# cyberfabric/cyberfabric-core

Hardware: NVIDIA H100
Metric: prompt_bytes_per_sec_bpe_encode (higher is better)
Workload: dtype u32

## Files before the change

### cyberfabric-core_b200/csrc/bpe_kernels.cuh

```cuda
#pragma once
#include <stdint.h>

#include "pretok.cuh"
#include "pretok_fsm.h"
#include "pretok_sync.cuh"
#include "specials.h"
#include "tables.h"
#include "tma.cuh"

namespace cfbpe {

#ifdef CUSIM_EMULATOR
#define CFBPE_DYN_SMEM(name) uint32_t* const name = reinterpret_cast<uint32_t*>(cusim::dyn_smem())
#else
#define CFBPE_DYN_SMEM(name) extern __shared__ __align__(16) uint32_t name[]
#endif

constexpr uint32_t kMaxVocabs = 8;
#ifdef CUSIM_EMULATOR
inline unsigned long long* dbg_counters() { static unsigned long long c[16]; return c; }
#define CFBPE_DBG_COUNT(i) (++dbg_counters()[i])
#else
#define CFBPE_DBG_COUNT(i) ((void)0)
#endif

#ifndef CFBPE_SPLIT_CHUNK
#define CFBPE_SPLIT_CHUNK 64
#endif
constexpr uint32_t kSplitChunk = CFBPE_SPLIT_CHUNK;
constexpr uint32_t kBigPiece = 256;
constexpr uint32_t kScanTileWords = 256;

struct VocabSet {
    TablesView v[kMaxVocabs];
    uint32_t loaded_mask;
};

struct BatchView {
    const uint8_t* bytes;
    const uint64_t* offsets;
    const uint8_t* vocab_ids;
    uint32_t n_prompts;
    uint64_t total_bytes;
};

struct DeviceStatus {
    uint32_t bad_utf8;
    uint32_t n_long;
    uint32_t long_overflow;
    uint32_t long_next;
    uint32_t n_big;
    uint32_t defer_next;
    uint64_t n_tokens;
    uint64_t tok_end;
    unsigned long long long_bytes;
    unsigned long long long_tokens;
    uint32_t miss_n[3];
    uint32_t miss_next[3];
    uint32_t miss_overflow;
    uint32_t extra_n;
    uint32_t split_next;
    uint32_t fix_n;
    uint32_t bad_vocab;
    uint32_t defer_n;
    unsigned long long defer_parts;
    uint64_t n_chunks;
    uint64_t chunk_end;
};

struct MissLists {
    uint64_t* list[3];
    uint32_t cap[3];
};
__host__ __device__ inline uint32_t miss_class_min_len(uint32_t c) { return c == 0 ? 13u : (c == 1 ? 7u : 1u); }

struct LongPiece { uint64_t start; uint64_t end; uint32_t vocab; uint32_t pad; };

__device__ __forceinline__ uint32_t find_prompt(const uint64_t* __restrict__ offsets, uint32_t n, uint64_t pos) {
    uint32_t lo = 0, hi = n;
    while (hi - lo > 1) {
        const uint32_t mid = (lo + hi) >> 1;
        if (offsets[mid] <= pos) lo = mid; else hi = mid;
    }
    return lo;
}

__device__ __forceinline__ void or_bits(uint32_t* __restrict__ words, uint64_t word, uint32_t bits) {
    if (bits) atomicOr(&words[word], bits);
}

__device__ __forceinline__ void prefetch_l2(const void* p) {
#if !defined(CUSIM_EMULATOR)
    asm volatile("prefetch.global.L2 [%0];" ::"l"(p));
#else
    (void)p;
#endif
}

__device__ __forceinline__ uint64_t same_byte_run_end(const uint8_t* __restrict__ s, uint64_t pos, uint64_t pe, uint32_t c) {
    uint64_t e = pos;
    while (e < pe && (reinterpret_cast<uintptr_t>(s + e) & 15u)) { if (s[e] != c) return e; ++e; }
    const uint32_t w = c * 0x01010101u;
    for (uint64_t a = e; a < pe && a < e + 1024; a += 128) prefetch_l2(s + a);
    while (e + 128 <= pe) {
        if (e + 1024 < pe) prefetch_l2(s + e + 1024);
        uint4 v[8];
// ... 513 lines not shown
    uint32_t* sid = &s_id[wic][0][lane];
    uint32_t* srk = &s_rk[wic][0][lane];
    if (status->miss_overflow) return;
    TablesView T = vs.v[0];
    uint32_t vid = 0;
#pragma unroll 1
    for (uint32_t c = 0; c < 3; ++c) {
        const uint32_t n = status->miss_n[c];
        const uint64_t* __restrict__ list = ml.list[c];
        for (;;) {
            uint32_t t0 = 0;
            if (lane == 0) t0 = atomicAdd(&status->miss_next[c], 32u);
            t0 = __shfl_sync(kFull, t0, 0);
            if (t0 >= n) break;
            const uint32_t i = t0 + lane;
            uint32_t alive = 0, rank = 0;
            if (i < n) {
                const uint64_t e = list[i];
                const uint64_t pos = e & 0xFFFFFFFFull;
                rank = static_cast<uint32_t>(e >> 32);
                const uint64_t end = next_set_bit(piece_bits, pos + 1, b.total_bytes);
                if (multi) {
                    const uint32_t pv = b.vocab_ids[find_prompt(b.offsets, b.n_prompts, pos)];
                    if (pv != vid) { vid = pv; T = vs.v[vid]; }
                }
                alive = merge_piece_in_lane(T, text, pos, static_cast<uint32_t>(end - pos), sid, srk, tok_bits);
            }
            const uint32_t cnt = __popc(alive);
            uint32_t incl = cnt;
#pragma unroll
            for (uint32_t d = 1; d < 32; d <<= 1) { const uint32_t o = __shfl_up_sync(kFull, incl, d); if (lane >= d) incl += o; }
            const uint32_t total = __shfl_sync(kFull, incl, 31);
            uint32_t base = 0;
            if (lane == 0 && total) base = atomicAdd(&status->extra_n, total);
            base = __shfl_sync(kFull, base, 0);
            if (cnt) {
                uint32_t slot = base + incl - cnt;
                if (slot + cnt <= dn.extras_cap) {
                    dn.by_piece[rank] = kPieceMulti | slot;
                    for (uint32_t bits = alive; bits; bits &= bits - 1) dn.extras[slot++] = sid[(static_cast<uint32_t>(__ffs(bits)) - 1u) * 32];
                } else atomicOr(&status->miss_overflow, 1u);
            }
            __syncwarp();
        }
    }
}

struct LongScratch {
    uint32_t* rank;
    uint32_t* aux0;
    uint32_t* aux1;
};

__device__ __forceinline__ uint32_t warp_min_u32(uint32_t v) {
#pragma unroll
    for (uint32_t d = 16; d; d >>= 1) { const uint32_t o = __shfl_xor_sync(kFull, v, d); v = o < v ? o : v; }
    return v;
}

__device__ __forceinline__ bool select_chunk(uint32_t r, uint32_t rmin, uint32_t lane, uint32_t& carry, uint32_t& sel_ballot) {
    const bool cand = (r == rmin);
    const uint32_t C = __ballot_sync(kFull, cand);
    const uint32_t z = ~C & lanemask_lt(lane);
    const uint32_t s = z ? (32u - __clz(z)) : 0u;
    const uint32_t cnt = lane - s + (s == 0 ? carry : 0u);
    const bool sel = cand && !(cnt & 1u);
    sel_ballot = __ballot_sync(kFull, sel);
    const uint32_t nz = ~C;
    carry = nz ? static_cast<uint32_t>(__clz(nz)) : (carry + 32u);
    return sel;
}

__device__ __forceinline__ void array_round(const TablesView& T, uint32_t* id, uint32_t* rk, uint32_t* a0, uint32_t* a1,
                                            uint32_t m, uint32_t rmin, uint32_t lane) {
    uint32_t carry = 0, prevS = 0, cut = kNone;
    for (uint32_t base = 0; base < m && cut == kNone; base += 32) {
        const uint32_t i = base + lane;
        const uint32_t r = (i + 1 < m) ? rk[i] : kNone;
        uint32_t S;
        const bool sel = select_chunk(r, rmin, lane, carry, S);
        bool viol = false;
        if (sel) {
            const bool selm2 = (lane >= 2) ? ((S >> (lane - 2)) & 1u) : ((prevS >> (30 + lane)) & 1u);
            uint32_t L = kNone, R = kNone;
            if (i > 0) L = pair_lookup(T, selm2 ? rmin : id[i - 1], rmin);
            if (i + 2 < m) R = pair_lookup(T, rmin, id[i + 2]);
            a0[i] = L;
            a1[i] = R;
            viol = (L < rmin) || (R < rmin);
        }
        const uint32_t V = __ballot_sync(kFull, viol);
        if (V) cut = base + (__ffs(V) - 1);
        prevS = S;
    }
    __syncwarp();
    carry = 0; prevS = 0;
    for (uint32_t base = 0; base < m && base <= cut; base += 32) {
        const uint32_t i = base + lane;
        const uint32_t r = (i + 1 < m) ? rk[i] : kNone;
        uint32_t S;
        const bool sel = select_chunk(r, rmin, lane, carry, S);
        const bool app = sel && i <= cut;
        const bool selm2 = (lane >= 2) ? ((S >> (lane - 2)) & 1u) : ((prevS >> (30 + lane)) & 1u);
        uint32_t L = kNone;
        if (app) {
            L = a0[i];
            id[i] = rmin;
            id[i + 1] = kNone;
            rk[i] = a1[i];
        }
        __syncwarp();
        if (app && i > 0) rk[selm2 ? i - 2 : i - 1] = L;
        __syncwarp();
        prevS = S;
    }
}
template <uint32_t kPosBits>
__device__ __forceinline__ uint32_t array_compact(uint32_t* id, uint32_t* rk, uint32_t m, uint32_t lane, uint32_t& rmin_out) {
    uint32_t out = 0, nmin = kNone;
    for (uint32_t base = 0; base < m; base += 32) {
        const uint32_t i = base + lane;
        const uint32_t myid = (i < m) ? id[i] : kNone;
        uint32_t myrk = (i < m) ? rk[i] : kNone;
        if (kPosBits && myrk != kNone) myrk >>= kPosBits;
        const bool keep = myid != kNone;
        const uint32_t K = __ballot_sync(kFull, keep);
        const uint32_t pos = out + __popc(K & lanemask_lt(lane));
        __syncwarp();
        if (keep) { id[pos] = myid; rk[pos] = myrk; nmin = myrk < nmin ? myrk : nmin; }
        out += __popc(K);
    }
    __syncwarp();
    rmin_out = warp_min_u32(nmin);
    return out;
}

constexpr uint32_t kListMax = 65535;
constexpr uint32_t kMedSmem = 256;

__device__ __forceinline__ bool key_less(uint32_t r1, uint32_t p1, uint32_t r2, uint32_t p2) { return r1 < r2 || (r1 == r2 && p1 < p2); }

__device__ __forceinline__ void list_rounds_multi(const TablesView& T, uint32_t* id, uint32_t* rk, uint32_t* link, uint32_t* nid,
                                                  uint32_t m, uint32_t lane) {
    constexpr uint32_t kNoPrev = 0xFFFFu;
    for (uint32_t i = lane; i < m; i += 32) {
        link[i] = ((i + 1) << 16) | (i ? i - 1 : kNoPrev);
        nid[i] = (i + 1 < m) ? id[i + 1] : kNone;
    }
    __syncwarp();
    const uint32_t c = ((m + 31) / 32) | 1u;
    const uint32_t lo = lane * c < m ? lane * c : m;
    const uint32_t hi = lo + c < m ? lo + c : m;
    for (;;) {
        uint32_t m1 = kNone, p1 = 0, m2 = kNone, p2 = 0;
        for (uint32_t xb = lo; xb < hi; xb += 16) {
            uint32_t v[16];
#pragma unroll
            for (uint32_t t = 0; t < 16; ++t) v[t] = (xb + t < hi) ? rk[xb + t] : kNone;
#pragma unroll
            for (uint32_t t = 0; t < 16; ++t) {
                if (v[t] < m1) { m2 = m1; p2 = p1; m1 = v[t]; p1 = xb + t; }
                else if (v[t] < m2) { m2 = v[t]; p2 = xb + t; }
            }
        }
        if (!__any_sync(kFull, m1 != kNone)) break;
        const bool valid = m1 != kNone;
        const uint32_t x = p1, r = m1;
        uint32_t j = 0, q = kNoPrev, k = m, L = kNone, R = kNone;
        if (valid) {
            const uint32_t li = link[x];
            j = li >> 16; q = li & 0xFFFFu;
            k = link[j] >> 16;
            const uint32_t idk = nid[j];
            const uint32_t idq = (q != kNoPrev) ? id[q] : 0u;
// ... 107 lines not shown
                if (R != kNone) Rk = (R << kPosBits) | x;
                if (L != kNone) Lk = (L << kPosBits) | q;
            }
            have = dirty != nullptr;
        }
        const bool valid = m1 != kNoKey;
        const uint32_t x = m1 & kPosMask, r = m1 >> kPosBits;
        uint32_t v = kNoKey;
        bool viol = false;
        if (valid) {
            uint32_t cc = m2 < Lk ? m2 : Lk;
            cc = cc < Rk ? cc : Rk;
            viol = cc <= m1;
            v = cc > m1 + 1u ? cc : m1 + 1u;
            if (v == kNoKey) v = kNoKey - 1u;
            atomicMin(&claim[x], m1);
            atomicMin(&claim[j], m1);
        }
        group_sync();
        if (kWarps > 1 && tid == 0) eq_flag[(round + 1u) & 1u] = 0;
        if (valid) {
            uint32_t lowest = claim[x];
            const uint32_t cj = claim[j];
            lowest = cj < lowest ? cj : lowest;
            if (q != kNoPrev) { const uint32_t cq = claim[q]; lowest = cq < lowest ? cq : lowest; }
            if (k < m) { const uint32_t ck = claim[k]; lowest = ck < lowest ? ck : lowest; }
            if (lowest < m1) { v = m1; have = false; }
        }
        uint32_t cut = __reduce_min_sync(kFull, v);
        if (kWarps > 1) {
            uint32_t* red = s_red + (round & 1u) * kWarps;
            if (lane == 0) red[wid] = cut;
            __syncthreads();
            cut = red[0];
#pragma unroll
            for (uint32_t w = 1; w < kWarps; ++w) { const uint32_t o = red[w]; cut = o < cut ? o : cut; }
        } else {
            __syncwarp();
        }
        if (cut == kNoKey) return true;
        if (kWarps > 1 && tid == 0) CFBPE_DBG_COUNT(6);
        if (kWarps > 1 && valid && m1 < cut) CFBPE_DBG_COUNT(7);
        bool eq = valid && m1 < cut && !viol && (cut >> kPosBits) == (m1 >> kPosBits);
        if (kWarps == 1) eq = __any_sync(kFull, eq);
        else if (eq) eq_flag[round & 1u] = 1u;
        if (valid) {
            claim[x] = kNoKey; claim[j] = kNoKey;
            if (m1 < cut) {
                id[x] = r; id[j] = kNone;
                kk[j] = kNoKey; kk[x] = Rk;
                link[x] = (k << 16) | q;
                if (k < m) link[k] = (link[k] & 0xFFFF0000u) | x;
                if (q != kNoPrev) kk[q] = Lk;
                have = false;
                if (dirty) {
                    if (j >= hi) dirty[(j * inv_c) >> 20] = 1u;
                    if (q != kNoPrev && q < lo) dirty[(q * inv_c) >> 20] = 1u;
                }
            }
        }
        group_sync();
        if (kWarps > 1) eq = eq_flag[round & 1u] != 0u;
        eq_run = eq ? eq_run + 1u : 0u;
        if (eq_run >= 3u) {
            const uint32_t er = cut >> kPosBits;
            uint32_t cnt = 0;
            for (uint32_t y = lo; y < hi; ++y) cnt += (kk[y] >> kPosBits) == er ? 1u : 0u;
            cnt = __reduce_add_sync(kFull, cnt);
            if (kWarps > 1) {
                uint32_t* sum = s_red + 2 * kWarps + 2;
                if (lane == 0) sum[wid] = cnt;
                __syncthreads();
                cnt = 0;
#pragma unroll
                for (uint32_t w = 0; w < kWarps; ++w) cnt += sum[w];
                __syncthreads();
            }
            if (cnt >= 8u && cnt * 32u >= m) return false;
            eq_run = 0;
        }
    }
}

__device__ __forceinline__ void flag_parts(const uint32_t* id, uint32_t* copy_to, uint32_t m, uint64_t start,
                                           uint32_t* __restrict__ tok_bits, DeviceStatus* status, uint32_t lane) {
    for (uint32_t base = 0; base < m; base += 32) {
        const uint32_t i = base + lane;
        const uint32_t v = (i < m) ? id[i] : kNone;
        const bool alive = v != kNone;
        if (alive && copy_to) copy_to[i] = v;
        const uint32_t A = __ballot_sync(kFull, alive);
        if (lane == 0 && A) {
            atomicAdd(&status->long_tokens, static_cast<unsigned long long>(__popc(A)));
            const uint64_t pos = start + base;
            const uint32_t sh = static_cast<uint32_t>(pos & 31);
            atomicOr(&tok_bits[pos >> 5], A << sh);
            if (sh && (A >> (32 - sh))) atomicOr(&tok_bits[(pos >> 5) + 1], A >> (32 - sh));
        }
    }
}

constexpr uint32_t kDeferMaxParts = 4096;
constexpr uint32_t kListSmemBytes = kDeferMaxParts * 16;
constexpr uint32_t kListMaxRank = (1u << 20) - 1u;
__device__ __forceinline__ bool list_kernel_takes(const TablesView& T, uint32_t n_bytes) { return n_bytes <= kDeferMaxParts && T.n_ranks < kListMaxRank; }


constexpr uint32_t kLongWarps = 4;
#ifndef CFBPE_LONG_MIN_CTAS
#define CFBPE_LONG_MIN_CTAS (32 / kLongWarps)
#endif
__global__ void __launch_bounds__(kLongWarps * 32, CFBPE_LONG_MIN_CTAS)
bpe_long_kernel(BatchView b, VocabSet vs, LongPiece* long_list, DeviceStatus* status,
                uint32_t long_cap, uint32_t* __restrict__ ids_by_pos, LongScratch sc, uint32_t* __restrict__ tok_bits) {
    __shared__ uint32_t s_med[kLongWarps][4][kMedSmem];
    const uint32_t lane = threadIdx.x & 31;
    const uint32_t n_big = status->n_big;
    const uint32_t n_all = status->long_overflow ? 0u : status->n_long + n_big;
    for (;;) {
        uint32_t item = 0;
        if (lane == 0) item = atomicAdd(&status->long_next, 1u);
        item = __shfl_sync(kFull, item, 0);
        if (item >= n_all) break;
        const uint32_t slot = item < n_big ? long_cap - 1 - item : item - n_big;
        const LongPiece lp = long_list[slot];
        const TablesView T = vs.v[lp.vocab];
        const uint8_t* __restrict__ p = b.bytes + lp.start;
        const uint32_t n = static_cast<uint32_t>(lp.end - lp.start);
#ifndef CFBPE_NO_DEFER
        if (item < n_big && list_kernel_takes(T, n)) continue;
#endif
        uint32_t* const gid = ids_by_pos + lp.start;
        const bool in_smem = n <= kMedSmem;
        uint32_t* id = in_smem ? s_med[threadIdx.x >> 5][0] : gid;
        uint32_t* rk = in_smem ? s_med[threadIdx.x >> 5][1] : sc.rank + lp.start;
        uint32_t* a0 = in_smem ? s_med[threadIdx.x >> 5][2] : sc.aux0 + lp.start;
        uint32_t* a1 = in_smem ? s_med[threadIdx.x >> 5][3] : sc.aux1 + lp.start;

        if (n <= T.max_token_len) {
            uint32_t t = kNone;
            if (lane == 0) t = piece_lookup(T, p, n);
            t = __shfl_sync(kFull, t, 0);
            if (t != kNone) {
                if (lane == 0) { gid[0] = t; atomicOr(&tok_bits[lp.start >> 5], 1u << (lp.start & 31)); atomicAdd(&status->long_tokens, 1ull); }
                continue;
            }
        }
        uint32_t m = n;
        uint32_t rmin = kNone;
        for (uint32_t i = lane; i < n; i += 32) {
            const uint32_t c0 = p[i];
            id[i] = T.byte2id[c0];
            const uint32_t r = (i + 1 < n) ? T.bytepair[(c0 << 8) | p[i + 1]] : kNone;
            rk[i] = r;
            rmin = r < rmin ? r : rmin;
        }
        rmin = warp_min_u32(rmin);
        __syncwarp();

        bool deferred = false;
        while (rmin != kNone) {
            array_round(T, id, rk, a0, a1, m, rmin, lane);
            const uint32_t before = m;
            m = array_compact<0>(id, rk, m, lane, rmin);
            const uint32_t merged = before - m;
            if (rmin == kNone || merged * 8u >= m || m <= 32u || m > kListMax) continue;
            if (in_smem) {
                if (list_rounds_par<1, 8>(T, id, rk, a0, a1, m, nullptr)) break;
                if (lane == 0) CFBPE_DBG_COUNT(1);
                m = array_compact<8>(id, rk, m, lane, rmin);
                continue;
            }
            if (lane == 0) CFBPE_DBG_COUNT(5);
            list_rounds_multi(T, id, rk, a0, a1, m, lane);
            __syncwarp();
            break;
        }
        if (deferred) continue;
        __syncwarp();
        flag_parts(id, in_smem ? gid : nullptr, m, lp.start, tok_bits, status, lane);
        __syncwarp();
    }
}

constexpr uint32_t kCtaChunk = 16;

__device__ __forceinline__ void cta_array_round(const TablesView& T, uint32_t* id, uint32_t* rk, uint32_t* a0, uint32_t* a1,
                                                uint32_t m, uint32_t rmin, uint32_t* s_scan, uint32_t* s_sel) {
    const uint32_t P = blockDim.x, t = threadIdx.x;
    const uint32_t c = (m + P - 1) / P;
    const uint32_t lo = t * c < m ? t * c : m, hi = lo + c < m ? lo + c : m;
    uint32_t tail = 0, all = 1;
    for (uint32_t i = lo; i < hi; ++i) {
        const bool cand = (i + 1 < m) && rk[i] == rmin;
        if (cand) ++tail; else { tail = 0; all = 0; }
    }
    s_scan[t] = (all << 31) | tail;
    if (t == 0) s_scan[P] = kNone;
    for (uint32_t w = t; w < kDeferMaxParts / 32; w += P) s_sel[w] = 0;
    __syncthreads();
    uint32_t cnt = 0;
    for (uint32_t u = t; u > 0 && lo < m;) {
        const uint32_t e = s_scan[--u];
        cnt += e & 0x7FFFFFFFu;
        if (!(e >> 31)) break;
    }
    uint32_t sel_bits = 0;
    for (uint32_t i = lo; i < hi; ++i) {
        const bool cand = (i + 1 < m) && rk[i] == rmin;
        if (cand && !(cnt & 1u)) { sel_bits |= 1u << (i - lo); atomicOr(&s_sel[i >> 5], 1u << (i & 31)); }
        cnt = cand ? cnt + 1 : 0;
    }
    __syncthreads();
    uint32_t m2_bits = 0;
    for (uint32_t bts = sel_bits; bts; bts &= bts - 1) {
        const uint32_t k = static_cast<uint32_t>(__ffs(bts)) - 1u, i = lo + k;
        const bool selm2 = i >= 2 && ((s_sel[(i - 2) >> 5] >> ((i - 2) & 31)) & 1u);
        uint32_t L = kNone, R = kNone;
        if (i > 0) L = pair_lookup(T, selm2 ? rmin : id[i - 1], rmin);
        if (i + 2 < m) R = pair_lookup(T, rmin, id[i + 2]);
        a0[i] = L; a1[i] = R;
        if (selm2) m2_bits |= 1u << k;
        if (L < rmin || R < rmin) atomicMin(&s_scan[P], i);
    }
    __syncthreads();
    const uint32_t cut = s_scan[P];
    for (uint32_t bts = sel_bits; bts; bts &= bts - 1) {
        const uint32_t i = lo + static_cast<uint32_t>(__ffs(bts)) - 1u;
        if (i > cut) break;
        id[i] = rmin; id[i + 1] = kNone; rk[i] = a1[i];
    }
    __syncthreads();
    for (uint32_t bts = sel_bits; bts; bts &= bts - 1) {
        const uint32_t k = static_cast<uint32_t>(__ffs(bts)) - 1u, i = lo + k;
        if (i > cut) break;
        if (i > 0) rk[((m2_bits >> k) & 1u) ? i - 2 : i - 1] = a0[i];
    }
    __syncthreads();
}

template <uint32_t kPosBits>
__device__ __forceinline__ uint32_t cta_array_compact(uint32_t* id, uint32_t* rk, uint32_t m, uint32_t& rmin_out, uint32_t* s_scan) {
    const uint32_t P = blockDim.x, t = threadIdx.x, lane = t & 31u, wid = t >> 5;
    const uint32_t c = (m + P - 1) / P;
    const uint32_t lo = t * c < m ? t * c : m, hi = lo + c < m ? lo + c : m;
    uint32_t vid[kCtaChunk], vrk[kCtaChunk];
    uint32_t keep = 0, nmin = kNone;
#pragma unroll
    for (uint32_t k = 0; k < kCtaChunk; ++k) {
        const uint32_t i = lo + k;
        vid[k] = (k < c && i < hi) ? id[i] : kNone;
        uint32_t r = (k < c && i < hi) ? rk[i] : kNone;
        if (kPosBits && r != kNone) r >>= kPosBits;
        vrk[k] = r;
        if (vid[k] != kNone) { ++keep; nmin = r < nmin ? r : nmin; }
    }
    uint32_t x = keep;
#pragma unroll
    for (uint32_t d = 1; d < 32; d <<= 1) { const uint32_t o = __shfl_up_sync(kFull, x, d); if (lane >= d) x += o; }
    nmin = warp_min_u32(nmin);
    if (lane == 31) s_scan[wid] = x;
    if (lane == 0) s_scan[32 + wid] = nmin;
    __syncthreads();
    uint32_t woff = 0, total = 0, rmin = kNone;
    for (uint32_t w = 0; w < (P >> 5); ++w) { const uint32_t v = s_scan[w]; if (w < wid) woff += v; total += v; const uint32_t r = s_scan[32 + w]; rmin = r < rmin ? r : rmin; }
    uint32_t pos = woff + x - keep;
#pragma unroll
    for (uint32_t k = 0; k < kCtaChunk; ++k) if (vid[k] != kNone) { id[pos] = vid[k]; rk[pos] = vrk[k]; ++pos; }
    __syncthreads();
    rmin_out = rmin;
    return total;
}

#ifndef CFBPE_LIST_WARPS
#define CFBPE_LIST_WARPS 8
#endif
constexpr uint32_t kListWarps = CFBPE_LIST_WARPS;
static_assert(kListWarps * 32 * kCtaChunk >= kDeferMaxParts, "a thread's chunk of the batched rounds holds kCtaChunk parts");

__global__ void __launch_bounds__(kListWarps * 32, 3)
bpe_list_kernel(BatchView b, VocabSet vs, const LongPiece* __restrict__ long_list, DeviceStatus* status,
                uint32_t long_cap, uint32_t* __restrict__ ids_by_pos, LongScratch sc, uint32_t* __restrict__ tok_bits) {
    CFBPE_DYN_SMEM(s_dyn);
    __shared__ uint32_t s_red[3 * kListWarps + 2];
    __shared__ uint32_t s_item, s_tok;
    __shared__ uint32_t s_dirty[kListWarps * 32];
    __shared__ uint32_t s_scan[kListWarps * 32 + 64];
    __shared__ uint32_t s_sel[kDeferMaxParts / 32];
    const uint32_t n_big = status->long_overflow ? 0u : status->n_big;
    uint32_t* const id = s_dyn;
    uint32_t* const kk = s_dyn + kDeferMaxParts;
    uint32_t* const link = s_dyn + 2 * kDeferMaxParts;
    uint32_t* const claim = s_dyn + 3 * kDeferMaxParts;
    (void)sc;
    for (;;) {
        if (threadIdx.x == 0) s_item = atomicAdd(&status->defer_next, 1u);
        __syncthreads();
        const uint32_t item = s_item;
        __syncthreads();
        if (item >= n_big) break;
        const LongPiece lp = long_list[long_cap - 1 - item];
        const TablesView T = vs.v[lp.vocab];
        const uint32_t n = static_cast<uint32_t>(lp.end - lp.start);
        if (!list_kernel_takes(T, n)) continue;
        const uint8_t* __restrict__ p = b.bytes + lp.start;
        uint32_t* const gid = ids_by_pos + lp.start;
        if (n <= T.max_token_len) {
            if (threadIdx.x == 0) s_tok = piece_lookup(T, p, n);
            __syncthreads();
            const uint32_t tok = s_tok;
            __syncthreads();
            if (tok != kNone) {
                if (threadIdx.x == 0) { gid[0] = tok; atomicOr(&tok_bits[lp.start >> 5], 1u << (lp.start & 31)); atomicAdd(&status->long_tokens, 1ull); }
                continue;
            }
        }
        uint32_t m = n, rmin = kNone;
        for (uint32_t i = threadIdx.x; i < n; i += kListWarps * 32) {
            const uint32_t c0 = p[i];
            id[i] = T.byte2id[c0];
            const uint32_t r = (i + 1 < n) ? T.bytepair[(c0 << 8) | p[i + 1]] : kNone;
            kk[i] = r;
            rmin = r < rmin ? r : rmin;
        }
        rmin = warp_min_u32(rmin);
        if ((threadIdx.x & 31) == 0) s_scan[threadIdx.x >> 5] = rmin;
        __syncthreads();
        rmin = kNone;
        for (uint32_t w = 0; w < kListWarps; ++w) { const uint32_t r = s_scan[w]; rmin = r < rmin ? r : rmin; }
        __syncthreads();
        bool counted = false;
        while (rmin != kNone) {
            cta_array_round(T, id, kk, link, claim, m, rmin, s_scan, s_sel);
            const uint32_t before = m;
            m = cta_array_compact<0>(id, kk, m, rmin, s_scan);
            if (rmin == kNone || (before - m) * 8u >= m || m <= 32u) continue;
            if (!counted && threadIdx.x == 0) { atomicAdd(&status->defer_n, 1u); atomicAdd(&status->defer_parts, static_cast<unsigned long long>(m)); CFBPE_DBG_COUNT(0); }
            counted = true;
            const bool done = list_rounds_par<kListWarps, 12>(T, id, kk, link, claim, m, s_red, s_dirty);
            __syncthreads();
            if (done) break;
            if (threadIdx.x == 0) CFBPE_DBG_COUNT(2);
            m = cta_array_compact<12>(id, kk, m, rmin, s_scan);
        }
        __syncthreads();
        if (threadIdx.x < 32) flag_parts(id, gid, m, lp.start, tok_bits, status, threadIdx.x);
        __syncthreads();
    }
}

__device__ __forceinline__ uint32_t block_reduce_add_256(uint32_t v, uint32_t* s_tmp) {
#pragma unroll
    for (uint32_t d = 16; d; d >>= 1) v += __shfl_xor_sync(kFull, v, d);
    if ((threadIdx.x & 31) == 0) s_tmp[threadIdx.x >> 5] = v;
    __syncthreads();
    uint32_t t = 0;
    for (uint32_t w = 0; w < (blockDim.x + 31) / 32; ++w) t += s_tmp[w];
    __syncthreads();
    return t;
}

__global__ void __launch_bounds__(256)
flag_count_kernel(uint32_t* __restrict__ tok_bits, const uint32_t* __restrict__ piece_bits, uint64_t n_words, uint32_t* __restrict__ tile_counts) {
    __shared__ uint32_t s_tmp[8];
    const uint64_t base = static_cast<uint64_t>(blockIdx.x) * kScanTileWords;
    uint32_t c = 0;
    for (uint32_t i = threadIdx.x; i < kScanTileWords; i += blockDim.x) {
        const uint64_t w = base + i;
        if (w < n_words) { const uint32_t t = tok_bits[w], f = t | piece_bits[w]; if (f != t) tok_bits[w] = f; c += __popc(f); }
    }
    const uint32_t t = block_reduce_add_256(c, s_tmp);
    if (threadIdx.x == 0) tile_counts[blockIdx.x] = t;
}

__global__ void __launch_bounds__(1024)
tile_scan_kernel(const uint32_t* __restrict__ tile_counts, uint32_t n_tiles, uint64_t* __restrict__ tile_base,
                 DeviceStatus* status, const uint64_t* __restrict__ token_base) {
    __shared__ uint64_t s_warp[32];
    const uint64_t base0 = token_base ? *token_base : 0;
    const uint32_t lane = threadIdx.x & 31, wid = threadIdx.x >> 5, nwarps = (blockDim.x + 31) >> 5;
    const uint32_t per = ((n_tiles + nwarps - 1) / nwarps + 31u) & ~31u;
    const uint32_t lo = wid * per < n_tiles ? wid * per : n_tiles;
    const uint32_t hi = lo + per < n_tiles ? lo + per : n_tiles;
    uint64_t sum = 0;
    for (uint32_t i = lo + lane; i < hi; i += 32) sum += tile_counts[i];
#pragma unroll
    for (uint32_t d = 16; d; d >>= 1) sum += __shfl_xor_sync(kFull, sum, d);
    if (lane == 0) s_warp[wid] = sum;
    __syncthreads();
    uint64_t carry = base0, total = 0;
    for (uint32_t w = 0; w < nwarps; ++w) { const uint64_t v = s_warp[w]; if (w < wid) carry += v; total += v; }
    for (uint32_t i0 = lo; i0 < hi; i0 += 32) {
        const uint32_t i = i0 + lane;
        const uint64_t v = i < hi ? tile_counts[i] : 0;
        uint64_t x = v;
#pragma unroll
        for (uint32_t d = 1; d < 32; d <<= 1) { const uint64_t o = __shfl_up_sync(kFull, x, d); if (lane >= d) x += o; }
        if (i < hi) tile_base[i] = carry + x - v;
        carry += __shfl_sync(kFull, x, 31);
    }
    if (threadIdx.x == 0 && status) { status->n_tokens = total; status->tok_end = base0 + total; }
}

__global__ void __launch_bounds__(256, 8)
emit_compact_kernel(const uint32_t* __restrict__ tok_bits, const uint32_t* __restrict__ piece_bits, uint64_t n_words,
                    const uint64_t* __restrict__ tile_base, DenseIds dn, const uint32_t* __restrict__ ids_by_pos,
                    uint32_t* __restrict__ out_ids, uint64_t out_cap) {
    constexpr uint32_t kWarps = kScanTileWords / 32;
    constexpr uint16_t kStart = 0x8000u;
    __shared__ uint32_t s_warp[kWarps], s_pw[kWarps];
    __shared__ uint16_t s_list[kWarps][32 * 32];
    const uint64_t w = static_cast<uint64_t>(blockIdx.x) * kScanTileWords + threadIdx.x;
    const uint64_t w0 = w - (threadIdx.x & 31);
    const uint32_t lane = threadIdx.x & 31, wid = threadIdx.x >> 5;
    const uint32_t bits = (w < n_words) ? tok_bits[w] : 0u;
    const uint32_t pb = (w < n_words) ? piece_bits[w] : 0u;
    uint32_t prev_bits = 0, prev_pb = 0;
    if (lane == 0 && w0 > 0 && w0 <= n_words) { prev_bits = tok_bits[w0 - 1]; prev_pb = piece_bits[w0 - 1]; }
    const uint64_t tok_tile = tile_base[blockIdx.x];
    const uint64_t piece_tile = (w0 < n_words) ? dn.piece_base[w0 >> 6] : 0u;
    const uint32_t c = __popc(bits), pc = __popc(pb);
    uint32_t x = c, px = pc;
#pragma unroll
    for (uint32_t d = 1; d < 32; d <<= 1) {
        const uint32_t o = __shfl_up_sync(kFull, x, d), po = __shfl_up_sync(kFull, px, d);
        if (lane >= d) { x += o; px += po; }
    }
    if (lane == 31) { s_warp[wid] = x; s_pw[wid] = px; }
    uint16_t* list = s_list[wid];
    for (uint32_t rest = bits, j = x - c; rest; rest &= rest - 1, ++j) {
// ... 391 lines not shown
```

### cyberfabric-core_b200/csrc/cfbpe.cu

```cuda
#include <cuda_runtime.h>

#include <chrono>
#include <cstdio>
#include <cstdlib>
#include <cstring>
#include <mutex>
#include <string>
#include <vector>

#include "../../include/cfbpe.h"

struct ProfEvents;
#define CFBPE_LAUNCH(kernel, grid, block, stream, ...) kernel<<<(grid), (block), 0, (stream)>>>(__VA_ARGS__)
#define CFBPE_LAUNCH_SMEM(kernel, grid, block, smem, stream, ...) kernel<<<(grid), (block), (smem), (stream)>>>(__VA_ARGS__)
#define CFBPE_ZERO(ptr, bytes, stream) cudaMemsetAsync((ptr), 0, (bytes), (stream))
#define CFBPE_MARK(prof, idx, stream, begin) prof_mark((prof), (idx), (stream), (begin))
static inline void prof_mark(ProfEvents* p, int idx, cudaStream_t s, bool begin);
#define CFBPE_FORK(main, aux, ev) do { if ((main) != (aux)) { cudaEventRecord((ev), (main)); cudaStreamWaitEvent((aux), (ev), 0); } } while (0)
#define CFBPE_JOIN(main, aux, ev) do { if ((main) != (aux)) { cudaEventRecord((ev), (aux)); cudaStreamWaitEvent((main), (ev), 0); } } while (0)

#include "pipeline.cuh"
#include "pretok_ctx.h"
#include "specials.cuh"
#include "subbatch.h"
// ... 1084 lines not shown
    CK(cudaStreamSynchronize(s));
    if (prof) fill_profile(ln, total_bytes);
    if (n_tokens) *n_tokens = ln->h_status->n_tokens;
    return device_call_status(ctx, ln);
}

int run_device(cfbpe_ctx* ctx, uint32_t n_prompts, const uint8_t* d_bytes, uint64_t total_bytes, const uint64_t* d_offsets,
               const uint8_t* d_vocab_ids, uint32_t* d_out_ids, uint32_t* d_out_starts, uint64_t out_cap, uint64_t* d_out_offsets,
               uint32_t* d_out_counts, uint64_t* n_tokens, void* stream) {
    return device_call(ctx, n_prompts, d_bytes, total_bytes, d_offsets, d_vocab_ids, d_out_offsets, d_out_ids != nullptr, out_cap, n_tokens, stream, true,
                       [&](DeviceCtx* dv, Lane* ln, const BatchView& b, cudaStream_t s, ProfEvents* prof) {
        enqueue_encode(b, dv->vs, dv->uc, ln->ws, d_out_ids, out_cap, d_out_offsets, d_out_counts,
                       static_cast<uint32_t>(dv->sm_count * 4), s, prof ? s : ln->aux_stream, prof ? s : ln->aux2_stream,
                       ln->ev_fork, ln->ev_join, ln->ev_join2, prof, nullptr, d_out_starts);
        CK(cudaGetLastError());
        return CFBPE_OK;
    });
}

int run_device_special(cfbpe_ctx* ctx, uint32_t n_prompts, const uint8_t* d_bytes, uint64_t total_bytes, const uint64_t* d_offsets,
                       const uint8_t* d_vocab_ids, const uint8_t* const* modes, uint32_t* d_out_ids, uint64_t out_cap, uint64_t* d_out_offsets,
                       uint32_t* d_out_counts, uint64_t* n_tokens, uint32_t* out_bad, void* stream) {
    return device_call(ctx, n_prompts, d_bytes, total_bytes, d_offsets, d_vocab_ids, d_out_offsets, d_out_ids != nullptr, out_cap, n_tokens, stream, false,
                       [&](DeviceCtx* dv, Lane* ln, const BatchView& b, cudaStream_t s, ProfEvents*) {
        SpecialSet sp;
        bool scan = false, spliced = false;
        const EncodeOut out{d_out_ids, out_cap, d_out_offsets, d_out_counts};
        int rc = special_set(ctx, dv, ln, modes, &sp, &scan, s);
        if (!rc) rc = enqueue_special_call(ctx, dv, ln, b, sp, scan, s, out, out, out_bad, &spliced);
        if (!rc && spliced) CK(cudaMemcpyAsync(&ln->ws.status->n_tokens, &ln->sp.status->fin.n_tokens, 2 * sizeof(uint64_t), cudaMemcpyDeviceToDevice, s));
        return rc;
    });
}

int run_device_truncate(cfbpe_ctx* ctx, uint32_t n_prompts, const uint8_t* d_bytes, uint64_t total_bytes, const uint64_t* d_offsets,
                        const uint8_t* d_vocab_ids, const uint32_t* d_budgets, uint32_t mode, uint32_t* d_out_cut, uint32_t* d_out_kept,
                        uint32_t* d_out_counts, void* stream) {
    return device_call(ctx, n_prompts, d_bytes, total_bytes, d_offsets, d_vocab_ids, d_out_cut, false, 0, nullptr, stream, true,
                       [&](DeviceCtx* dv, Lane* ln, const BatchView& b, cudaStream_t s, ProfEvents* prof) {
        const TruncateView tv{d_budgets, mode == CFBPE_TRUNCATE_TAIL ? 1u : 0u, d_out_cut, d_out_kept};
        enqueue_encode(b, dv->vs, dv->uc, ln->ws, ln->d_out_ids, ctx->max_bytes, ln->d_out_offsets, d_out_counts,
                       static_cast<uint32_t>(dv->sm_count * 4), s, prof ? s : ln->aux_stream, prof ? s : ln->aux2_stream,
                       ln->ev_fork, ln->ev_join, ln->ev_join2, prof, nullptr, nullptr, &tv);
        CK(cudaGetLastError());
        return CFBPE_OK;
    });
}

int run_device_chunk(cfbpe_ctx* ctx, uint32_t n_prompts, const uint8_t* d_bytes, uint64_t total_bytes, const uint64_t* d_offsets,
                     const uint8_t* d_vocab_ids, uint32_t chunk_tokens, uint32_t overlap_tokens, uint32_t* d_out_spans, uint64_t chunk_cap,
                     uint64_t* d_out_chunk_offsets, uint32_t* d_out_counts, uint64_t* n_chunks, void* stream) {
    return device_call(ctx, n_prompts, d_bytes, total_bytes, d_offsets, d_vocab_ids, d_out_chunk_offsets, true, chunk_cap, n_chunks, stream, true,
                       [&](DeviceCtx* dv, Lane* ln, const BatchView& b, cudaStream_t s, ProfEvents* prof) {
        if (const int rc = ensure_starts_lane(ctx, ln)) return rc;
        const ChunkView cv{chunk_tokens, chunk_tokens - overlap_tokens, d_out_chunk_offsets, nullptr, d_out_spans, d_out_spans + 1, 2u, chunk_cap};
        enqueue_encode(b, dv->vs, dv->uc, ln->ws, ln->d_out_ids, ctx->max_bytes, ln->d_out_offsets, d_out_counts,
                       static_cast<uint32_t>(dv->sm_count * 4), s, prof ? s : ln->aux_stream, prof ? s : ln->aux2_stream,
                       ln->ev_fork, ln->ev_join, ln->ev_join2, prof, nullptr, ln->d_out_starts, nullptr, &cv);
        CK(cudaGetLastError());
        static_assert(offsetof(DeviceStatus, chunk_end) == offsetof(DeviceStatus, n_chunks) + sizeof(uint64_t) &&
                      offsetof(DeviceStatus, tok_end) == offsetof(DeviceStatus, n_tokens) + sizeof(uint64_t), "count, then end");
        CK(cudaMemcpyAsync(&ln->ws.status->n_tokens, &ln->ws.status->n_chunks, 2 * sizeof(uint64_t), cudaMemcpyDeviceToDevice, s));
        return CFBPE_OK;
    });
}

}

struct DeviceGuard {
    int prev = -1;
    DeviceGuard() { if (cudaGetDevice(&prev) != cudaSuccess) { prev = -1; cudaGetLastError(); } }
    ~DeviceGuard() { if (prev >= 0) cudaSetDevice(prev); }
};

extern "C" {

int cfbpe_abi_version(void) { return static_cast<int>(CFBPE_ABI_VERSION); }

#ifndef CFBPE_SRC_HASH
#define CFBPE_SRC_HASH "unknown"
#endif
const char* cfbpe_build_id(void) { return CFBPE_SRC_HASH; }

int cfbpe_create(const cfbpe_config* cfg, cfbpe_ctx** out) {
    DeviceGuard restore_device;
    if (!cfg || !out || cfg->struct_size < offsetof(cfbpe_config, devices)) return CFBPE_EINVAL;
    *out = nullptr;
    int ndev = 0;
    if (cudaGetDeviceCount(&ndev) != cudaSuccess || ndev == 0) return CFBPE_ENODEV;
    const bool has_multi = cfg->struct_size >= sizeof(cfbpe_config);
    std::vector<int> devices;
    if (has_multi && cfg->n_devices > 0) {
        if (cfg->n_devices > CFBPE_MAX_DEVICES) return CFBPE_EINVAL;
        for (uint32_t i = 0; i < cfg->n_devices; ++i) devices.push_back(cfg->devices[i]);
    } else devices.push_back(cfg->device);
    for (size_t i = 0; i < devices.size(); ++i) {
        if (devices[i] < 0 || devices[i] >= ndev) return CFBPE_ENODEV;
        for (size_t j = 0; j < i; ++j) if (devices[j] == devices[i]) return CFBPE_EINVAL;
    }
    cfbpe_ctx* ctx = new (std::nothrow) cfbpe_ctx();
    if (!ctx) return CFBPE_ENOMEM;
    ctx->max_bytes = cfg->max_batch_bytes ? cfg->max_batch_bytes : (256ull << 20);
    ctx->max_prompts = cfg->max_prompts ? cfg->max_prompts : (1u << 20);
    ctx->n_workspaces = (has_multi && cfg->n_workspaces) ? cfg->n_workspaces : 1u;
    if (ctx->max_bytes >= (1ull << 32) - 4096 || ctx->n_workspaces > 16) { delete ctx; return CFBPE_EINVAL; }
    if (devices.size() > 1 && !load_nccl(&ctx->nccl)) { delete ctx; tl_err = "a multi-device context needs libnccl.so.2 (vocabulary broadcast, gather of the shard totals)"; return CFBPE_EIO; }
    for (size_t i = 0; i < devices.size(); ++i) {
        ctx->devs.emplace_back(new DeviceCtx());
        if (!create_device(ctx->devs.back().get(), devices[i], static_cast<int>(i), ctx->n_workspaces, ctx->max_bytes, ctx->max_prompts)) {
            const bool nodev = ctx->devs.back()->sm_count == 0;
            cudaGetLastError();
            cfbpe_destroy(ctx);
            return nodev ? CFBPE_ENODEV : CFBPE_ENOMEM;
        }
    }
    if (devices.size() > 1) {
        std::vector<void*> comms(devices.size(), nullptr);
        const int rc = ctx->nccl.CommInitAll(comms.data(), static_cast<int>(devices.size()), devices.data());
        if (rc != 0) { tl_err = std::string("ncclCommInitAll: ") + ctx->nccl.GetErrorString(rc); cfbpe_destroy(ctx); return CFBPE_EIO; }
        for (size_t i = 0; i < devices.size(); ++i) ctx->devs[i]->comm = comms[i];
        bool peers = std::getenv("CFBPE_NO_PEER") == nullptr;
        for (size_t a = 0; a < devices.size() && peers; ++a) {
            cudaSetDevice(devices[a]);
            for (size_t b2 = 0; b2 < devices.size() && peers; ++b2) {
                if (a == b2) continue;
                int can = 0;
                if (cudaDeviceCanAccessPeer(&can, devices[a], devices[b2]) != cudaSuccess || !can) { peers = false; break; }
                const cudaError_t e = cudaDeviceEnablePeerAccess(devices[b2], 0);
                if (e != cudaSuccess && e != cudaErrorPeerAccessAlreadyEnabled) peers = false;
                cudaGetLastError();
            }
        }
        ctx->peer_ok = peers;
    }
    if (const char* e = std::getenv("CFBPE_PIPE_CHUNK_BYTES")) { const uint64_t v = std::strtoull(e, nullptr, 10); if (v >= 1024) ctx->pipe_chunk = v; }
    if (const char* e = std::getenv("CFBPE_PIPE_MIN_BYTES")) { const uint64_t v = std::strtoull(e, nullptr, 10); if (v >= 1) ctx->pipe_min = v; }
    *out = ctx;
    return CFBPE_OK;
}

void cfbpe_destroy(cfbpe_ctx* ctx) {
    DeviceGuard restore_device;
    if (!ctx) return;
    for (auto& dvp : ctx->devs) {
        DeviceCtx* dv = dvp.get();
        cudaSetDevice(dv->device);
        cudaDeviceSynchronize();
        if (dv->comm && ctx->nccl.CommDestroy) ctx->nccl.CommDestroy(dv->comm);
        for (auto& ln : dv->lanes) destroy_lane(ln.get());
        cudaSetDevice(dv->device);
        cudaFree(dv->d_uc1); cudaFree(dv->d_uc2); cudaFree(dv->d_ascii); cudaFree(dv->d_fsm); cudaFree(dv->d_split_tables);
        for (auto& v : dv->vocabs) { if (v.d_blob) cudaFree(v.d_blob); }
        for (auto* t : dv->d_specials) cudaFree(t);
    }
    delete ctx;
}

const char* cfbpe_last_error(const cfbpe_ctx*) { return tl_err.c_str(); }

int cfbpe_vocab_load(cfbpe_ctx* ctx, uint32_t vocab_id, const uint8_t* ranks_file, size_t len, uint32_t format,
                     uint32_t pattern_id, uint32_t max_ranks) {
    DeviceGuard restore_device;
    if (!ctx) return CFBPE_EINVAL;
    tl_err.clear();
    if (vocab_id >= CFBPE_MAX_VOCABS) return fail(ctx, CFBPE_EINVAL, "vocab_id out of range");
    if (!ranks_file || !len) return fail(ctx, CFBPE_EINVAL, "empty rank file");
// ... 287 lines not shown
```

Baseline: 35.98 billion.

## Prefetch next long-piece ticket and overlap whole-piece hash probe with byte init

The long and list kernels now fetch the next work ticket and its LongPiece record before processing the current piece, hiding the atomic and load latency. The whole-piece vocabulary lookup is split into a begin step (hash plus first slot load) and a warp-cooperative finish step, placed so it overlaps the byte-to-id initialization. Pair lookups use a combined pair_lookup2, and flag_parts now returns its token count so the global atomic is done once per piece, spread across warps in the list kernel. Optional per-piece clock instrumentation and emulator counters are added behind macros. The speculative initialization does wasted work when the probe hits, and the double-buffered shared state adds complexity.

```diff
diff --git a/cyberfabric-core_b200/csrc/bpe_kernels.cuh b/cyberfabric-core_b200/csrc/bpe_kernels.cuh
--- a/cyberfabric-core_b200/csrc/bpe_kernels.cuh
+++ b/cyberfabric-core_b200/csrc/bpe_kernels.cuh
@@ -20,8 +20,10 @@
 #ifdef CUSIM_EMULATOR
 inline unsigned long long* dbg_counters() { static unsigned long long c[16]; return c; }
 #define CFBPE_DBG_COUNT(i) (++dbg_counters()[i])
+#define CFBPE_DBG_ADD(i, v) (dbg_counters()[i] += (v))
 #else
 #define CFBPE_DBG_COUNT(i) ((void)0)
+#define CFBPE_DBG_ADD(i, v) ((void)0)
 #endif
 
 #ifndef CFBPE_SPLIT_CHUNK
@@ -701,14 +703,14 @@
         bool viol = false;
         if (sel) {
             const bool selm2 = (lane >= 2) ? ((S >> (lane - 2)) & 1u) : ((prevS >> (30 + lane)) & 1u);
-            uint32_t L = kNone, R = kNone;
-            if (i > 0) L = pair_lookup(T, selm2 ? rmin : id[i - 1], rmin);
-            if (i + 2 < m) R = pair_lookup(T, rmin, id[i + 2]);
+            uint32_t L, R;
+            pair_lookup2(T, i > 0 ? (selm2 ? rmin : id[i - 1]) : 0u, rmin, i > 0, rmin, i + 2 < m ? id[i + 2] : 0u, i + 2 < m, L, R);
             a0[i] = L;
             a1[i] = R;
             viol = (L < rmin) || (R < rmin);
         }
         const uint32_t V = __ballot_sync(kFull, viol);
+        if (lane == 0 && S) CFBPE_DBG_COUNT(14);
         if (V) cut = base + (__ffs(V) - 1);
         prevS = S;
     }
@@ -982,23 +984,115 @@
     }
 }
 
-__device__ __forceinline__ void flag_parts(const uint32_t* id, uint32_t* copy_to, uint32_t m, uint64_t start,
-                                           uint32_t* __restrict__ tok_bits, DeviceStatus* status, uint32_t lane) {
-    for (uint32_t base = 0; base < m; base += 32) {
+__device__ __forceinline__ uint32_t flag_parts(const uint32_t* id, uint32_t* copy_to, uint32_t m, uint64_t start,
+                                               uint32_t* __restrict__ tok_bits, uint32_t lane, uint32_t first = 0, uint32_t step = 32) {
+    uint32_t tokens = 0;
+    for (uint32_t base = first; base < m; base += step) {
         const uint32_t i = base + lane;
         const uint32_t v = (i < m) ? id[i] : kNone;
         const bool alive = v != kNone;
         if (alive && copy_to) copy_to[i] = v;
         const uint32_t A = __ballot_sync(kFull, alive);
         if (lane == 0 && A) {
-            atomicAdd(&status->long_tokens, static_cast<unsigned long long>(__popc(A)));
+            tokens += __popc(A);
             const uint64_t pos = start + base;
             const uint32_t sh = static_cast<uint32_t>(pos & 31);
             atomicOr(&tok_bits[pos >> 5], A << sh);
             if (sh && (A >> (32 - sh))) atomicOr(&tok_bits[(pos >> 5) + 1], A >> (32 - sh));
         }
     }
-}
+    return tokens;
+}
+
+#if defined(CFBPE_PIECE_CLOCK) && !defined(CUSIM_EMULATOR)
+constexpr uint32_t kPieceClockCap = 1u << 18;
+struct PieceClock {
+    unsigned long long t0, t1;
+    uint32_t c[6];
+    uint32_t n, rounds;
+    uint32_t sm, kind;
+};
+__device__ PieceClock g_piece_clock[kPieceClockCap];
+__device__ unsigned int g_piece_clock_n;
+struct PieceClockRun {
+    long long s = 0, m = 0;
+    unsigned long long g0 = 0;
+    uint32_t c[6] = {0, 0, 0, 0, 0, 0}, nb = 0, nl = 0;
+    __device__ __forceinline__ void start() { s = clock64(); asm volatile("mov.u64 %0, %%globaltimer;" : "=l"(g0)); nb = nl = 0; c[3] = c[4] = 0; }
+    __device__ __forceinline__ void at(int k) { c[k] = static_cast<uint32_t>(clock64() - s); }
+    __device__ __forceinline__ void begin() { m = clock64(); }
+    __device__ __forceinline__ void batched() { c[3] += static_cast<uint32_t>(clock64() - m); ++nb; }
+    __device__ __forceinline__ void list() { c[4] += static_cast<uint32_t>(clock64() - m); ++nl; }
+    __device__ __forceinline__ void write(uint32_t n, uint32_t kind) {
+        c[5] = static_cast<uint32_t>(clock64() - s);
+        unsigned long long g1; asm volatile("mov.u64 %0, %%globaltimer;" : "=l"(g1));
+        uint32_t sm; asm volatile("mov.u32 %0, %%smid;" : "=r"(sm));
+        const uint32_t k = atomicAdd(&g_piece_clock_n, 1u);
+        if (k >= kPieceClockCap) return;
+        PieceClock& r = g_piece_clock[k];
+        r.t0 = g0; r.t1 = g1;
+        for (int i = 0; i < 6; ++i) r.c[i] = c[i];
+        r.n = n; r.rounds = nb | (nl << 16); r.sm = sm; r.kind = kind;
+    }
+};
+#else
+struct PieceClockRun {
+    __device__ __forceinline__ void start() {}
+    __device__ __forceinline__ void at(int) {}
+    __device__ __forceinline__ void begin() {}
+    __device__ __forceinline__ void batched() {}
+    __device__ __forceinline__ void list() {}
+    __device__ __forceinline__ void write(uint32_t, uint32_t) {}
+};
+#endif
+
+struct LongProbe { uint64_t hash; uint32_t h; LongSlot s; };
+__device__ __forceinline__ LongProbe long_probe_begin(const TablesView& T, const uint8_t* p, uint32_t n) {
+    uint64_t k0; uint32_t k1;
+    pack_key(p, n, k0, k1);
+    LongProbe q;
+    q.hash = long_hash(k0, k1, load_le32(p + n - 4), n);
+    q.h = static_cast<uint32_t>(q.hash >> 17) & T.long_mask;
+    q.s = T.lng[q.h];
+    return q;
+}
+__device__ __forceinline__ uint32_t long_probe_finish(const TablesView& T, LongProbe q, const uint8_t* p, uint32_t n, uint32_t lane) {
+    for (;;) {
+        const uint32_t meta = __shfl_sync(kFull, q.s.meta, 0);
+        if (meta == kMetaEmpty) return kNone;
+        if (__shfl_sync(kFull, (q.s.hash == q.hash && (meta >> 24) == (n & 0xFF)) ? 1u : 0u, 0)) {
+            const uint32_t id = meta & 0x00FFFFFFu;
+            if (T.tokoff[id + 1] - T.tokoff[id] == n) {
+                const uint8_t* tok = T.blob + __shfl_sync(kFull, q.s.blob_off, 0);
+                bool eq = true;
+                for (uint32_t o = lane * 4; o < n; o += 128) {
+                    const uint32_t at = o + 4 <= n ? o : n - 4;
+                    eq = eq && load_u32_any(tok + at) == load_u32_any(p + at);
+                }
+                if (__all_sync(kFull, eq)) return id;
+            }
+        }
+        if (lane == 0) { q.h = (q.h + 1) & T.long_mask; q.s = T.lng[q.h]; }
+    }
+}
+
+#ifdef CUSIM_EMULATOR
+inline uint32_t long_probe_extra_trips(const TablesView& t, const uint8_t* p, uint32_t len) {
+    uint64_t k0; uint32_t k1;
+    pack_key(p, len, k0, k1);
+    const uint64_t hash = long_hash(k0, k1, load_le32(p + len - 4), len);
+    uint32_t h = static_cast<uint32_t>(hash >> 17) & t.long_mask, trips = 0;
+    for (;; ++trips, h = (h + 1) & t.long_mask) {
+        const LongSlot s = t.lng[h];
+        if (s.meta == kMetaEmpty) return trips;
+        if (s.hash == hash && (s.meta >> 24) == (len & 0xFF)) {
+            const uint32_t id = s.meta & 0x00FFFFFFu;
+            ++trips;
+            if (t.tokoff[id + 1] - t.tokoff[id] == len) { ++trips; if (bytes_equal(t.blob + s.blob_off, p, len)) return trips; }
+        }
+    }
+}
+#endif
 
 constexpr uint32_t kDeferMaxParts = 4096;
 constexpr uint32_t kListSmemBytes = kDeferMaxParts * 16;
@@ -1017,19 +1111,38 @@
     const uint32_t lane = threadIdx.x & 31;
     const uint32_t n_big = status->n_big;
     const uint32_t n_all = status->long_overflow ? 0u : status->n_long + n_big;
-    for (;;) {
-        uint32_t item = 0;
-        if (lane == 0) item = atomicAdd(&status->long_next, 1u);
-        item = __shfl_sync(kFull, item, 0);
-        if (item >= n_all) break;
-        const uint32_t slot = item < n_big ? long_cap - 1 - item : item - n_big;
-        const LongPiece lp = long_list[slot];
+    PieceClockRun pc;
+    auto ticket = [&]() { uint32_t t = 0; if (lane == 0) t = atomicAdd(&status->long_next, 1u); return t; };
+    auto record = [&](uint32_t it) {
+        uint32_t w = 0;
+        if (it < n_all && lane < sizeof(LongPiece) / 4)
+            w = reinterpret_cast<const uint32_t*>(long_list + (it < n_big ? long_cap - 1 - it : it - n_big))[lane];
+        return w;
+    };
+    uint32_t item = __shfl_sync(kFull, ticket(), 0);
+    uint32_t rec = record(item);
+    if (lane == 0) CFBPE_DBG_ADD(11, item < n_all ? 2 : 1);
+    while (item < n_all) {
+        pc.start();
+        const uint32_t next = ticket();
+        const uint32_t cur = item;
+        LongPiece lp;
+        lp.start = __shfl_sync(kFull, rec, 0) | (static_cast<uint64_t>(__shfl_sync(kFull, rec, 1)) << 32);
+        lp.end = __shfl_sync(kFull, rec, 2) | (static_cast<uint64_t>(__shfl_sync(kFull, rec, 3)) << 32);
+        lp.vocab = __shfl_sync(kFull, rec, 4);
+        auto take_next = [&](uint32_t hidden) {
+            item = __shfl_sync(kFull, next, 0);
+            rec = record(item);
+            const uint32_t trips = item < n_all ? 2u : 1u;
+            if (lane == 0) CFBPE_DBG_ADD(11, trips - (hidden < trips ? hidden : trips));
+        };
         const TablesView T = vs.v[lp.vocab];
         const uint8_t* __restrict__ p = b.bytes + lp.start;
         const uint32_t n = static_cast<uint32_t>(lp.end - lp.start);
 #ifndef CFBPE_NO_DEFER
-        if (item < n_big && list_kernel_takes(T, n)) continue;
+        if (cur < n_big && list_kernel_takes(T, n)) { take_next(0); continue; }
 #endif
+        pc.at(0);
         uint32_t* const gid = ids_by_pos + lp.start;
         const bool in_smem = n <= kMedSmem;
         uint32_t* id = in_smem ? s_med[threadIdx.x >> 5][0] : gid;
@@ -1037,48 +1150,67 @@
         uint32_t* a0 = in_smem ? s_med[threadIdx.x >> 5][2] : sc.aux0 + lp.start;
         uint32_t* a1 = in_smem ? s_med[threadIdx.x >> 5][3] : sc.aux1 + lp.start;
 
-        if (n <= T.max_token_len) {
-            uint32_t t = kNone;
-            if (lane == 0) t = piece_lookup(T, p, n);
-            t = __shfl_sync(kFull, t, 0);
+        const bool probe = n <= T.max_token_len;
+        uint32_t t = kNone;
+        LongProbe q{};
+        if (probe && lane == 0) {
+            q = long_probe_begin(T, p, n);
+            CFBPE_DBG_ADD(12, 1 + long_probe_extra_trips(T, p, n));
+        }
+        if (probe && !in_smem) t = long_probe_finish(T, q, p, n, lane);
+        pc.at(1);
+        uint32_t m = n;
+        uint32_t rmin = kNone;
+        if (t == kNone) {
+            for (uint32_t i = lane; i < n; i += 32) {
+                const uint32_t c0 = p[i];
+                id[i] = T.byte2id[c0];
+                const uint32_t r = (i + 1 < n) ? T.bytepair[(c0 << 8) | p[i + 1]] : kNone;
+                rk[i] = r;
+                rmin = r < rmin ? r : rmin;
+            }
+        }
+        if (probe && in_smem) t = long_probe_finish(T, q, p, n, lane);
+        rmin = warp_min_u32(rmin);
+        __syncwarp();
+        if (probe) {
             if (t != kNone) {
-                if (lane == 0) { gid[0] = t; atomicOr(&tok_bits[lp.start >> 5], 1u << (lp.start & 31)); atomicAdd(&status->long_tokens, 1ull); }
+                if (lane == 0) { gid[0] = t; atomicOr(&tok_bits[lp.start >> 5], 1u << (lp.start & 31)); atomicAdd(&status->long_tokens, 1ull); CFBPE_DBG_COUNT(15); }
+                if (lane == 0) { pc.at(2); pc.write(n, 0x101u); }
+                take_next(1);
                 continue;
             }
         }
-        uint32_t m = n;
-        uint32_t rmin = kNone;
-        for (uint32_t i = lane; i < n; i += 32) {
-            const uint32_t c0 = p[i];
-            id[i] = T.byte2id[c0];
-            const uint32_t r = (i + 1 < n) ? T.bytepair[(c0 << 8) | p[i + 1]] : kNone;
-            rk[i] = r;
-            rmin = r < rmin ? r : rmin;
-        }
-        rmin = warp_min_u32(rmin);
-        __syncwarp();
-
-        bool deferred = false;
+        if (lane == 0) CFBPE_DBG_ADD(13, 2);
+        take_next(2);
+        pc.at(2);
+
         while (rmin != kNone) {
+            pc.begin();
             array_round(T, id, rk, a0, a1, m, rmin, lane);
             const uint32_t before = m;
             m = array_compact<0>(id, rk, m, lane, rmin);
+            pc.batched();
             const uint32_t merged = before - m;
             if (rmin == kNone || merged * 8u >= m || m <= 32u || m > kListMax) continue;
+            pc.begin();
             if (in_smem) {
-                if (list_rounds_par<1, 8>(T, id, rk, a0, a1, m, nullptr)) break;
+                if (list_rounds_par<1, 8>(T, id, rk, a0, a1, m, nullptr)) { pc.list(); break; }
                 if (lane == 0) CFBPE_DBG_COUNT(1);
                 m = array_compact<8>(id, rk, m, lane, rmin);
+                pc.list();
                 continue;
             }
             if (lane == 0) CFBPE_DBG_COUNT(5);
             list_rounds_multi(T, id, rk, a0, a1, m, lane);
             __syncwarp();
+            pc.list();
             break;
         }
-        if (deferred) continue;
         __syncwarp();
-        flag_parts(id, in_smem ? gid : nullptr, m, lp.start, tok_bits, status, lane);
+        const uint32_t nt = flag_parts(id, in_smem ? gid : nullptr, m, lp.start, tok_bits, lane);
+        if (lane == 0 && nt) { atomicAdd(&status->long_tokens, static_cast<unsigned long long>(nt)); CFBPE_DBG_COUNT(15); }
+        if (lane == 0) pc.write(n, 1u);
         __syncwarp();
     }
 }
@@ -1116,9 +1248,9 @@
     for (uint32_t bts = sel_bits; bts; bts &= bts - 1) {
         const uint32_t k = static_cast<uint32_t>(__ffs(bts)) - 1u, i = lo + k;
         const bool selm2 = i >= 2 && ((s_sel[(i - 2) >> 5] >> ((i - 2) & 31)) & 1u);
-        uint32_t L = kNone, R = kNone;
-        if (i > 0) L = pair_lookup(T, selm2 ? rmin : id[i - 1], rmin);
-        if (i + 2 < m) R = pair_lookup(T, rmin, id[i + 2]);
+        uint32_t L, R;
+        pair_lookup2(T, i > 0 ? (selm2 ? rmin : id[i - 1]) : 0u, rmin, i > 0, rmin, i + 2 < m ? id[i + 2] : 0u, i + 2 < m, L, R);
+        CFBPE_DBG_COUNT(14);
         a0[i] = L; a1[i] = R;
         if (selm2) m2_bits |= 1u << k;
         if (L < rmin || R < rmin) atomicMin(&s_scan[P], i);
@@ -1183,38 +1315,56 @@
                 uint32_t long_cap, uint32_t* __restrict__ ids_by_pos, LongScratch sc, uint32_t* __restrict__ tok_bits) {
     CFBPE_DYN_SMEM(s_dyn);
     __shared__ uint32_t s_red[3 * kListWarps + 2];
-    __shared__ uint32_t s_item, s_tok;
+    __shared__ uint32_t s_item[2], s_tok[2], s_ntok;
     __shared__ uint32_t s_dirty[kListWarps * 32];
     __shared__ uint32_t s_scan[kListWarps * 32 + 64];
     __shared__ uint32_t s_sel[kDeferMaxParts / 32];
     const uint32_t n_big = status->long_overflow ? 0u : status->n_big;
+    const uint32_t lane = threadIdx.x & 31;
     uint32_t* const id = s_dyn;
     uint32_t* const kk = s_dyn + kDeferMaxParts;
     uint32_t* const link = s_dyn + 2 * kDeferMaxParts;
     uint32_t* const claim = s_dyn + 3 * kDeferMaxParts;
     (void)sc;
-    for (;;) {
-        if (threadIdx.x == 0) s_item = atomicAdd(&status->defer_next, 1u);
-        __syncthreads();
-        const uint32_t item = s_item;
-        __syncthreads();
-        if (item >= n_big) break;
-        const LongPiece lp = long_list[long_cap - 1 - item];
+    PieceClockRun pc;
+    auto record = [&](uint32_t it) {
+        uint32_t w = 0;
+        if (it < n_big && lane < sizeof(LongPiece) / 4) w = reinterpret_cast<const uint32_t*>(long_list + (long_cap - 1 - it))[lane];
+        return w;
+    };
+    if (threadIdx.x == 0) { s_item[0] = atomicAdd(&status->defer_next, 1u); s_ntok = 0; }
+    __syncthreads();
+    uint32_t item = s_item[0], par = 1;
+    uint32_t rec = record(item);
+    if (threadIdx.x == 0) CFBPE_DBG_ADD(11, item < n_big ? 2 : 1);
+    while (item < n_big) {
+        pc.start();
+        uint32_t next = 0;
+        if (threadIdx.x == 0) next = atomicAdd(&status->defer_next, 1u);
+        LongPiece lp;
+        lp.start = __shfl_sync(kFull, rec, 0) | (static_cast<uint64_t>(__shfl_sync(kFull, rec, 1)) << 32);
+        lp.end = __shfl_sync(kFull, rec, 2) | (static_cast<uint64_t>(__shfl_sync(kFull, rec, 3)) << 32);
+        lp.vocab = __shfl_sync(kFull, rec, 4);
         const TablesView T = vs.v[lp.vocab];
         const uint32_t n = static_cast<uint32_t>(lp.end - lp.start);
-        if (!list_kernel_takes(T, n)) continue;
+        if (!list_kernel_takes(T, n)) {
+            if (threadIdx.x == 0) s_item[par] = next;
+            __syncthreads();
+            item = s_item[par]; par ^= 1u;
+            rec = record(item);
+            if (threadIdx.x == 0) CFBPE_DBG_ADD(11, item < n_big ? 2 : 1);
+            continue;
+        }
+        pc.at(0);
         const uint8_t* __restrict__ p = b.bytes + lp.start;
         uint32_t* const gid = ids_by_pos + lp.start;
-        if (n <= T.max_token_len) {
-            if (threadIdx.x == 0) s_tok = piece_lookup(T, p, n);
-            __syncthreads();
-            const uint32_t tok = s_tok;
-            __syncthreads();
-            if (tok != kNone) {
-                if (threadIdx.x == 0) { gid[0] = tok; atomicOr(&tok_bits[lp.start >> 5], 1u << (lp.start & 31)); atomicAdd(&status->long_tokens, 1ull); }
-                continue;
-            }
-        }
+        const bool probe = n <= T.max_token_len;
+        LongProbe q{};
+        if (probe && threadIdx.x == 0) {
+            q = long_probe_begin(T, p, n);
+            CFBPE_DBG_ADD(12, 1 + long_probe_extra_trips(T, p, n));
+        }
+        pc.at(1);
         uint32_t m = n, rmin = kNone;
         for (uint32_t i = threadIdx.x; i < n; i += kListWarps * 32) {
             const uint32_t c0 = p[i];
@@ -1223,29 +1373,54 @@
             kk[i] = r;
             rmin = r < rmin ? r : rmin;
         }
+        if (probe && threadIdx.x < 32) {
+            const uint32_t t = long_probe_finish(T, q, p, n, lane);
+            if (threadIdx.x == 0) s_tok[par] = t;
+        }
         rmin = warp_min_u32(rmin);
-        if ((threadIdx.x & 31) == 0) s_scan[threadIdx.x >> 5] = rmin;
+        if (lane == 0) s_scan[threadIdx.x >> 5] = rmin;
+        if (threadIdx.x == 0) s_item[par] = next;
         __syncthreads();
         rmin = kNone;
         for (uint32_t w = 0; w < kListWarps; ++w) { const uint32_t r = s_scan[w]; rmin = r < rmin ? r : rmin; }
+        const uint32_t tok = probe ? s_tok[par] : kNone;
+        item = s_item[par]; par ^= 1u;
         __syncthreads();
+        rec = record(item);
+        if (tok != kNone) {
+            if (threadIdx.x == 0) { gid[0] = tok; atomicOr(&tok_bits[lp.start >> 5], 1u << (lp.start & 31)); atomicAdd(&status->long_tokens, 1ull); CFBPE_DBG_COUNT(15); }
+            if (threadIdx.x == 0) { pc.at(2); pc.write(n, 0x102u); CFBPE_DBG_ADD(11, item < n_big ? 1 : 0); }
+            continue;
+        }
+        if (threadIdx.x == 0) CFBPE_DBG_ADD(13, 2);
+        pc.at(2);
         bool counted = false;
         while (rmin != kNone) {
+            pc.begin();
             cta_array_round(T, id, kk, link, claim, m, rmin, s_scan, s_sel);
             const uint32_t before = m;
             m = cta_array_compact<0>(id, kk, m, rmin, s_scan);
+            pc.batched();
             if (rmin == kNone || (before - m) * 8u >= m || m <= 32u) continue;
+            pc.begin();
             if (!counted && threadIdx.x == 0) { atomicAdd(&status->defer_n, 1u); atomicAdd(&status->defer_parts, static_cast<unsigned long long>(m)); CFBPE_DBG_COUNT(0); }
             counted = true;
             const bool done = list_rounds_par<kListWarps, 12>(T, id, kk, link, claim, m, s_red, s_dirty);
             __syncthreads();
-            if (done) break;
+            if (done) { pc.list(); break; }
             if (threadIdx.x == 0) CFBPE_DBG_COUNT(2);
             m = cta_array_compact<12>(id, kk, m, rmin, s_scan);
+            pc.list();
         }
         __syncthreads();
-        if (threadIdx.x < 32) flag_parts(id, gid, m, lp.start, tok_bits, status, threadIdx.x);
+        const uint32_t nt = flag_parts(id, gid, m, lp.start, tok_bits, lane, (threadIdx.x >> 5) * 32, kListWarps * 32);
+        if (lane == 0 && nt) atomicAdd(&s_ntok, nt);
         __syncthreads();
+        if (threadIdx.x == 0) {
+            if (s_ntok) { atomicAdd(&status->long_tokens, static_cast<unsigned long long>(s_ntok)); CFBPE_DBG_COUNT(15); }
+            s_ntok = 0;
+            pc.write(n, 2u);
+        }
     }
 }
 
diff --git a/cyberfabric-core_b200/csrc/cfbpe.cu b/cyberfabric-core_b200/csrc/cfbpe.cu
--- a/cyberfabric-core_b200/csrc/cfbpe.cu
+++ b/cyberfabric-core_b200/csrc/cfbpe.cu
@@ -1190,6 +1190,17 @@
 #endif
 const char* cfbpe_build_id(void) { return CFBPE_SRC_HASH; }
 
+#ifdef CFBPE_PIECE_CLOCK
+CFBPE_API long long cfbpe_piece_clock_read(void* out, unsigned cap) {
+    unsigned int n = 0, zero = 0;
+    if (cudaDeviceSynchronize() != cudaSuccess || cudaMemcpyFromSymbol(&n, g_piece_clock_n, sizeof(n)) != cudaSuccess) return -1;
+    const unsigned int k = n < cap ? (n < kPieceClockCap ? n : kPieceClockCap) : cap;
+    if (k && cudaMemcpyFromSymbol(out, g_piece_clock, k * sizeof(PieceClock)) != cudaSuccess) return -1;
+    if (cudaMemcpyToSymbol(g_piece_clock_n, &zero, sizeof(zero)) != cudaSuccess) return -1;
+    return n;
+}
+#endif
+
 int cfbpe_create(const cfbpe_config* cfg, cfbpe_ctx** out) {
     DeviceGuard restore_device;
     if (!cfg || !out || cfg->struct_size < offsetof(cfbpe_config, devices)) return CFBPE_EINVAL;
```

Measured after the change: 36.75 billion, median of 6. 2.1% higher.
